# yakir1991/LoRa-SDR-Lightweight-Standalone-Library-

Hardware: AMD Instinct MI355X
Metric: Msymbols/s dechirp+FFT+argmax @ SF7 & SF12, 1/2/4/8 GPU; % HBM roofline (higher is better)
Workload: dtype f32; 1 GPU; SF7 BW125 osr1 LEGACY lora_demodulate + fused dechirp, 15625 frames x (2 sync + 64 data) symbols per GPU, noiseless; launch=eager, streams=3, sf=7, osr=1, frames_per_gpu=15625, data_symbols_per_frame=64, parallelism=frames sharded x1, no collective (gloo timing only), symbols_ok=True

## Files before the change

lora-sdr-lightweight-standalone-library-_amd/csrc/lora_demod_fast.hip:

```cpp
#include "../../include/lora_mi355x.h"
#include "lora_internal.h"

#include <algorithm>
#include <cstdlib>
#include <type_traits>
#include <utility>

#pragma clang fp contract(off)

namespace lora {
namespace {


template <int SF>
struct Geo {
  static constexpr int N = 1 << SF;
  static constexpr bool SMALL = SF <= 5;
  static constexpr int P = SMALL ? N : 16;
  static constexpr int T = N / P;
  static constexpr int R1 = SMALL ? N : ((SF & 1) ? 8 : 16);
  static constexpr int LOGR1 = SMALL ? SF : ((SF & 1) ? 3 : 4);
  static constexpr int G1 = P / R1;
  static constexpr bool R2FIRST = (SF & 1) != 0;
  static constexpr int X = N / R1;
// ... 468 lines not shown
    case 0: return cf{1.0f, 0.0f};
    case 1: return cf{C1, -S1};
    case 2: return cf{R2, -R2};
    case 3: return cf{S1, -C1};
    case 4: return cf{0.0f, -1.0f};
    case 5: return cf{-S1, -C1};
    case 6: return cf{-R2, -R2};
    case 7: return cf{-C1, -S1};
    case 8: return cf{-1.0f, 0.0f};
    default: return cf{-C1, S1};
  }
}
template <int N>
struct ConstTw1 {
  __device__ __forceinline__ cf operator[](int i) const { return w16(i / (N / 16)); }
};

template <int SF, bool KEEP, bool FMA = false, bool TWL = false, bool PACK = false, bool CPRE = false,
          class HOOK = NoHook, bool FOLD = false>
__device__ __forceinline__ uint64_t fft_key(cf* z, cf* row, int l, const KArgs& a, float* second = nullptr,
                                            const cf* twl = nullptr, const int* cpre = nullptr, HOOK hook = HOOK{},
                                            const cf* wbpre = nullptr, const cf* wfold = nullptr) {
  using G = Geo<SF>;
  constexpr int N = G::N, T = G::T, P = G::P, R1 = G::R1;
  constexpr bool WL = G::WAVE_LOCAL;
  static_assert(!FOLD || FMA, "the folded rotation is the certified path's");
#pragma unroll
  for (int h = 0; h < G::G1; ++h) {
    if constexpr (FOLD) {
      cf* x = z + h * R1;
      const cf* w = wfold + h * R1;
      if constexpr (G::R2FIRST) {
#pragma unroll
        for (int b = 0; b < R1; b += 2) bfly2<true>(x[b], x[b + 1], w[b + 1]);
      } else {
#pragma unroll
        for (int b = 0; b < R1; b += 4) bfly4<true>(x[b], x[b + 1], x[b + 2], x[b + 3], w[b + 1], w[b + 2], w[b + 3]);
      }
      pass_regs<R1, G::R2FIRST, N, 1, !KEEP, FMA, ConstTw1<N>, true>(x, 0, ConstTw1<N>{});
    } else if constexpr (FMA) {
      pass_regs<R1, G::R2FIRST, N, 1, !KEEP, FMA, ConstTw1<N>>(z + h * R1, 0, ConstTw1<N>{});
    } else {
      pass_regs<R1, G::R2FIRST, N, 1, !KEEP, FMA>(z + h * R1, 0, a.tw);
    }
  }
  uint64_t key = 0;
  if constexpr (G::NPASS == 1) {
    float best = 0.0f;
    uint32_t bi = 0;
#pragma unroll
    for (int u = 0; u < R1; ++u) {
      const float m2 = z[u].re * z[u].re + z[u].im * z[u].im;
      if (m2 > best) {
        best = m2;
        bi = (uint32_t)u;
      }
    }
    key = ((uint64_t)__float_as_uint(best) << 32) | (uint32_t)(~bi);
  } else {
    int c[G::G1];
#pragma unroll
    for (int h = 0; h < G::G1; ++h) c[h] = CPRE ? cpre[h] : (int)(a.rev[l + T * h] >> G::LOGR1);
#pragma unroll
    for (int h = 0; h < G::G1; ++h)
#pragma unroll
      for (int u = 0; u < R1; ++u)
        row[lds_slot<SF>(c[h] * R1) + u] = z[h * R1 + u];
    block_sync<WL>();
    constexpr int RL = G::NPASS == 2 ? G::RA : G::RB;
    constexpr int ML = G::NPASS == 2 ? G::MA_A : G::MA_B;
    const cf* twA = TWL ? twl : a.twTA;
    if constexpr (G::NPASS == 2) {
      pass_lds<G::RA, N, G::MA_A, SF, T, P, true, FMA, false, TWL, PACK>(row, z, l, a.tw, key, twA, second);
    } else {
      pass_lds<G::RA, N, G::MA_A, SF, T, P, false, FMA, false, TWL>(row, z, l, a.tw, key, twA);
      block_sync<WL>();
      write_pass<G::RA, G::MA_A, SF, T, P>(row, z, l);
      block_sync<WL>();
      if constexpr (!std::is_same_v<HOOK, NoHook>) {
        const cf* wb = wbpre;
        __builtin_amdgcn_sched_barrier(0);
        hook();
        __builtin_amdgcn_sched_barrier(0);
        pass_lds<G::RB, N, G::MA_B, SF, T, P, true, FMA, true, TWL, PACK>(row, z, l, a.tw, key, a.twTB2, second, wb);
      } else {
        pass_lds<G::RB, N, G::MA_B, SF, T, P, true, FMA, true, TWL, PACK>(row, z, l, a.tw, key, a.twTB2, second);
      }
    }
    if constexpr (KEEP) {
      block_sync<WL>();
#pragma unroll
      for (int gg = 0; gg < P / RL; ++gg)
#pragma unroll
        for (int u = 0; u < RL; ++u) row[lds_slot<SF>(l + T * gg) + lds_slot<SF>(ML * u)] = z[gg * RL + u];
      block_sync<WL>();
    }
  }
  return key;
}

template <int SF, bool KEEP>
__device__ __forceinline__ void fft_key2(cf* z0, cf* z1, cf* row0, cf* row1, int l, const KArgs& a,
                                         uint64_t& k0, uint64_t& k1) {
  using G = Geo<SF>;
  static_assert(G::NPASS == 2 && G::WAVE_LOCAL, "wave-local two-pass transforms only");
  constexpr int N = G::N, T = G::T, P = G::P, R1 = G::R1;
#pragma unroll
  for (int h = 0; h < G::G1; ++h) {
    pass_regs<R1, G::R2FIRST, N, 1, !KEEP>(z0 + h * R1, 0, a.tw);
    pass_regs<R1, G::R2FIRST, N, 1, !KEEP>(z1 + h * R1, 0, a.tw);
  }
  int c[G::G1];
#pragma unroll
  for (int h = 0; h < G::G1; ++h) c[h] = (int)(a.rev[l + T * h] >> G::LOGR1);
#pragma unroll
  for (int h = 0; h < G::G1; ++h)
#pragma unroll
    for (int u = 0; u < R1; ++u) {
      row0[lds_slot<SF>(c[h] * R1) + u] = z0[h * R1 + u];
      row1[lds_slot<SF>(c[h] * R1) + u] = z1[h * R1 + u];
    }
  wave_sync();
  pass_lds<G::RA, N, G::MA_A, SF, T, P, true>(row0, z0, l, a.tw, k0, a.twTA);
  pass_lds<G::RA, N, G::MA_A, SF, T, P, true>(row1, z1, l, a.tw, k1, a.twTA);
  if constexpr (KEEP) {
    wave_sync();
#pragma unroll
    for (int gg = 0; gg < P / G::RA; ++gg)
#pragma unroll
      for (int u = 0; u < G::RA; ++u) {
        row0[lds_slot<SF>(l + T * gg) + lds_slot<SF>(G::MA_A * u)] = z0[gg * G::RA + u];
        row1[lds_slot<SF>(l + T * gg) + lds_slot<SF>(G::MA_A * u)] = z1[gg * G::RA + u];
      }
    wave_sync();
  }
}

template <int SF>
__device__ __forceinline__ uint64_t symbol_key(uint64_t key, int tid, uint64_t* red) {
  constexpr int T = Geo<SF>::T;
  if constexpr (T <= 64) {
    return group_max(key, T);
  } else {
    key = group_max(key, 64);
    __syncthreads();
    if ((tid & 63) == 0) red[tid >> 6] = key;
    __syncthreads();
    constexpr int WPS = T / 64;
    const int wb = ((tid >> 6) / WPS) * WPS;
    uint64_t r = red[wb];
#pragma unroll
    for (int q = 1; q < WPS; ++q) r = umax64(r, red[wb + q]);
    return r;
  }
}

__device__ __forceinline__ float amax3(float m, cf v) {
  asm("v_max3_f32 %0, %0, |%1|, |%2|" : "+v"(m) : "v"(v.re), "v"(v.im));
  return m;
}

template <int SF>
__device__ __forceinline__ void group_reduce2(float& a, float& b, int tid, float* rf) {
  constexpr int T = Geo<SF>::T;
  constexpr int W = T < 64 ? T : 64;
#pragma unroll
  for (int o = W >> 1; o > 0; o >>= 1) {
    a = fmaxf(a, __shfl_xor(a, o, 64));
    b = fmaxf(b, __shfl_xor(b, o, 64));
  }
  if constexpr (T > 64) {
    const int w = tid >> 6;
    if ((tid & 63) == 0) {
      rf[2 * w] = a;
      rf[2 * w + 1] = b;
    }
    __syncthreads();
    constexpr int WPS = T / 64;
    const int wb = (w / WPS) * WPS;
    a = rf[2 * wb];
    b = rf[2 * wb + 1];
#pragma unroll
    for (int q = 1; q < WPS; ++q) {
      a = fmaxf(a, rf[2 * (wb + q)]);
      b = fmaxf(b, rf[2 * (wb + q) + 1]);
    }
  }
}

__device__ __forceinline__ void top2_merge(uint32_t& b, uint32_t& s, uint32_t& p, uint32_t b2, uint32_t s2,
                                           uint32_t p2) {
  const uint32_t lo = b < b2 ? b : b2;
  const uint32_t hs = s > s2 ? s : s2;
  s = hs > lo ? hs : lo;
  b = b > b2 ? b : b2;
  p = p > p2 ? p : p2;
}
template <int O>
__device__ __forceinline__ uint32_t dpp_xchg(uint32_t v) {
  constexpr int ctrl = O == 1 ? 0xB1 : O == 2 ? 0x4E : O == 4 ? 0x141 : 0x140;
  return (uint32_t)__builtin_amdgcn_mov_dpp((int)v, ctrl, 0xF, 0xF, true);
}
template <int O, int W>
__device__ __forceinline__ void spec_reduce_step(uint32_t& best, uint32_t& sec, uint32_t& pm) {
  if constexpr (O < W) {
    if constexpr (O <= 8) {
      top2_merge(best, sec, pm, dpp_xchg<O>(best), dpp_xchg<O>(sec), dpp_xchg<O>(pm));
    } else if constexpr (O == 16) {
      const auto xb = __builtin_amdgcn_permlane16_swap(best, best, false, false);
      const auto xs = __builtin_amdgcn_permlane16_swap(sec, sec, false, false);
      const auto xp = __builtin_amdgcn_permlane16_swap(pm, pm, false, false);
      best = xb[0], sec = xs[0], pm = xp[0];
      top2_merge(best, sec, pm, xb[1], xs[1], xp[1]);
    } else {
      static_assert(O == 32, "wave64");
      const auto xb = __builtin_amdgcn_permlane32_swap(best, best, false, false);
      const auto xs = __builtin_amdgcn_permlane32_swap(sec, sec, false, false);
      const auto xp = __builtin_amdgcn_permlane32_swap(pm, pm, false, false);
      best = xb[0], sec = xs[0], pm = xp[0];
      top2_merge(best, sec, pm, xb[1], xs[1], xp[1]);
    }
    spec_reduce_step<2 * O, W>(best, sec, pm);
  }
}
template <int SF>
__device__ __forceinline__ void spec_reduce(uint32_t& best, uint32_t& sec, float& pmf, int tid, uint32_t* scratch) {
  constexpr int T = Geo<SF>::T;
  uint32_t pm = __float_as_uint(pmf);
  spec_reduce_step<1, (T < 64 ? T : 64)>(best, sec, pm);
  if constexpr (T > 64) {
    const int w = tid >> 6;
    if ((tid & 63) == 0) {
      scratch[3 * w] = best;
      scratch[3 * w + 1] = sec;
      scratch[3 * w + 2] = pm;
    }
    __syncthreads();
    constexpr int WPS = T / 64;
    const int wb = (w / WPS) * WPS;
    best = scratch[3 * wb];
    sec = scratch[3 * wb + 1];
    pm = scratch[3 * wb + 2];
#pragma unroll
    for (int q = 1; q < WPS; ++q)
      top2_merge(best, sec, pm, scratch[3 * (wb + q)], scratch[3 * (wb + q) + 1], scratch[3 * (wb + q) + 2]);
  }
  pmf = __uint_as_float(pm);
}

template <int SF>
constexpr int demod_waves_per_eu() {
  return SF >= 6 ? 4 : 1;
}

template <int SF, bool SPEC>
constexpr int demod_twl_entries() {
  if constexpr (!SPEC || SF < 6) {
    return 0;
  } else {
    using G = Geo<SF>;
    return (G::RA == 16 ? 15 : 3) * G::MA_A;
  }
}


template <int SF>
constexpr size_t spec_dtl_offset() {
  return (((size_t)Geo<SF>::SPW * lds_row<SF>() + demod_twl_entries<SF, true>()) * sizeof(cf) + 15) & ~(size_t)15;
}
template <int SF>
constexpr bool spec_dtab() {
  return Geo<SF>::WAVE_LOCAL && Geo<SF>::NPASS == 2 &&
         4 * (spec_dtl_offset<SF>() + 2 * sizeof(cf) * Geo<SF>::N) <= 160 * 1024;
}
template <int SF>
constexpr size_t spec_lds_bytes() {
  constexpr bool pf2 = Geo<SF>::WAVE_LOCAL && Geo<SF>::NPASS == 2;
  return pf2 ? spec_dtl_offset<SF>() + (spec_dtab<SF>() ? 2 * sizeof(cf) * Geo<SF>::N : 16 * 8 * Geo<SF>::T)
             : sizeof(cf) * ((size_t)Geo<SF>::SPW * lds_row<SF>() + demod_twl_entries<SF, true>());
}

#define LORA_SPEC_BLOCKS(SPB, dblocks, frames, sync) ((dblocks) + ((sync) ? (2 * (frames) + (SPB) - 1) / (SPB) : 0))
template <int SF>
struct SpecGrid {
  static constexpr int SPB = Geo<SF>::WAVE_LOCAL ? 64 / Geo<SF>::T : Geo<SF>::SPW;
  static constexpr int BPG = Geo<SF>::WAVE_LOCAL ? 4 : 1;
  __host__ __device__ static constexpr int bpf(int per) { return (per + SPB - 1) / SPB; }
  static constexpr int64_t groups(int64_t frames, int per, bool sync) {
    return (LORA_SPEC_BLOCKS(SPB, frames * bpf(per), frames, sync) + BPG - 1) / BPG;
  }
};

__device__ __forceinline__ __amdgpu_buffer_rsrc_t raw_rsrc(const void* p) {
  return __builtin_amdgcn_make_buffer_rsrc(const_cast<void*>(p), (short)0, 0x7fffffff, 0x00020000);
}

struct SpecBlk {
  int64_t f, base;
  int s, jl, d, cg;
  bool valid, mis, nbr;
  float rate;
  int toff;
};
template <int SF, int SPM, int DW, bool RECIP>
__device__ __forceinline__ void spec_decode(const KArgs& a, int64_t bb, int bpf, int per, int gi, int l, bool fdiv,
                                            uint64_t mq, SpecBlk& B) {
  constexpr int SPB = SpecGrid<SF>::SPB, S0 = SPM == 2 ? 0 : 2;
  const __attribute__((address_space(4))) FrameParams* fps =
      (const __attribute__((address_space(4))) FrameParams*)a.fp_spec;
  if constexpr (RECIP)
    B.f = fdiv ? (bpf == 1 ? bb : (int64_t)(((uint64_t)(uint32_t)bb * mq) >> 32)) : bb / bpf;
  else
    B.f = bb / bpf;
  B.jl = (int)(bb - B.f * bpf) * SPB + gi;
  B.valid = B.jl < per;
  B.s = S0 + (B.valid ? B.jl : per - 1);
  B.rate = SPM == 2 ? 0.0f : fps[B.f].rate;
  B.toff = SPM == 2 ? 0 : fps[B.f].t_off;
  sym_base(B.s, Geo<SF>::N, a.frame_len, B.toff, B.base, B.cg);
  if constexpr (SPM == 1) B.cg = 0;
  B.d = (int)(B.base & (DW - 1));
  B.mis = __builtin_amdgcn_readfirstlane(__ballot(Geo<SF>::NPASS == 3 ? l < B.d : B.d != 0) != 0);
  B.nbr = false;
}
template <int SF>
__device__ __forceinline__ bool spec_next_is_neighbour(const KArgs& a, const SpecBlk& B, int per, int gi) {
  int64_t bnext;
  int cgn;
  sym_base(B.s + 1, Geo<SF>::N, a.frame_len, B.toff, bnext, cgn);
  return gi < SpecGrid<SF>::SPB - 1 && B.jl + 1 < per && bnext == B.base + Geo<SF>::N;
}

template <int SF, bool DTAB, bool DTL>
__device__ __forceinline__ float4 spec_table_pair(int pp, __amdgpu_buffer_rsrc_t rd, int vt, bool cg0, const cf* dq,
                                                  const float4* dl) {
  constexpr int N = Geo<SF>::N, T = Geo<SF>::T;
  if constexpr (DTAB) {
    const cf d0 = dq[2 * pp * T], d1 = dq[(2 * pp + 1) * T];
    return float4{d0.re, d0.im, d1.re, d1.im};
  } else if constexpr (DTL) {
    return cg0 ? dl[pp * T]
               : __builtin_bit_cast(float4, __builtin_amdgcn_raw_buffer_load_b128(rd, vt, pp * (N + T) * 16, 0));
  } else {
    return __builtin_bit_cast(float4, __builtin_amdgcn_raw_buffer_load_b128(rd, vt, pp * (N + T) * 16, 0));
  }
}
template <int SF, bool DTAB, bool DTL, int NP>
__device__ __forceinline__ void spec_table(const KArgs& a, int cg, int lr, const cf* dtab, const float4* dtl,
                                           float4 (&dt)[NP]) {
  const __amdgpu_buffer_rsrc_t rd = raw_rsrc(a.downP);
  const int vt = (cg + lr) * 16;
  bool cg0 = false;
  if constexpr (DTL && !DTAB) cg0 = __builtin_amdgcn_readfirstlane(__ballot(cg != 0) == 0);
#pragma unroll
  for (int pp = 0; pp < NP; ++pp) dt[pp] = spec_table_pair<SF, DTAB, DTL>(pp, rd, vt, cg0, dtab + cg + lr, dtl + lr);
}
template <int MODE, bool MAX, int P>
__device__ __forceinline__ float spec_dechirp_max(const v2f (&ld)[P + 1], const float4* dt, cf (&in)[P]) {
#pragma unroll
  for (int q = 0; q < P; ++q) in[q] = cf{ld[q].x, ld[q].y};
  if constexpr (MODE == 0) {
#pragma unroll
    for (int pp = 0; pp < P / 2; ++pp) {
      in[2 * pp] = pk_cmul_ref(in[2 * pp], cf{dt[pp].x, dt[pp].y});
      in[2 * pp + 1] = pk_cmul_ref(in[2 * pp + 1], cf{dt[pp].z, dt[pp].w});
    }
  }
  float pm = 0.0f;
  if constexpr (MAX) {
#pragma unroll
    for (int q = 0; q < P; ++q) pm = amax3(pm, in[q]);
  }
  return pm;
}

__device__ __forceinline__ float spec_margin(uint32_t best, uint32_t sec) {
  return __builtin_amdgcn_sqrtf(spec_key_value(best)) - __builtin_amdgcn_sqrtf(spec_key_value(sec));
}
template <int SF, int S0>
__device__ __forceinline__ void spec_store_symbol(const KArgs& a, int64_t f, int s, int l, int lr, uint32_t lbest,
                                                  uint32_t best, uint32_t sec, float pm) {
  using G = Geo<SF>;
  constexpr int NG = G::NPASS == 2 ? G::P / G::RA : G::P / G::RB;
  constexpr int ML = G::NPASS == 2 ? G::MA_A : G::MA_B;
  const int o = (int)(best & 15u);
  const uint32_t idx = (uint32_t)(lr + G::T * (o % NG) + ML * (o / NG));
  const float margin = spec_margin(best, sec);
  if (lbest == best && a.syms) a.syms[f * a.sym_stride + (s - S0)] = (uint16_t)idx;
  if (l == 0)
    reinterpret_cast<uint2*>(a.spec_marg)[f * a.total + s] = make_uint2(__float_as_uint(margin), __float_as_uint(pm));
}

template <int SF, int MODE, bool FAST = false, bool SPEC = false>
__global__ void __launch_bounds__(256) __attribute__((amdgpu_waves_per_eu(demod_waves_per_eu<SF>())))
k_demod_fast(KArgs a, int s0, int64_t work, int rowc) {
  using G = Geo<SF>;
  constexpr int N = G::N, T = G::T, P = G::P, SPW = G::SPW;
  constexpr bool RAW = MODE == 3;
  constexpr bool DYN = MODE >= 2;
  extern __shared__ __attribute__((aligned(16))) unsigned char smem[];
  __shared__ uint64_t red[4];
  cf* rows = reinterpret_cast<cf*>(smem);
  const int tid = threadIdx.x;
  const int per = a.total - s0;
  const int step = DYN ? a.step : N;
  const int osr = DYN ? a.osr : 1;
  const bool legacy = RAW ? true : DYN ? a.mode != LORA_MODE_API : true;
  const bool dech = DYN ? (legacy && a.dechirp) : (MODE == 0);
  const bool hann = DYN ? (a.hann != 0) : false;

  const int g = tid / T;
  const int l = tid % T;
  const int64_t w0 = (int64_t)blockIdx.x * SPW;
  const int64_t f0 = w0 / per;
  const int r0 = (int)(w0 - f0 * per);
  const int64_t w = w0 + g;
  const bool valid = w < work;
  const int loc = r0 + (int)((valid ? w : work - 1) - w0);
  const int q = per >= SPW ? (loc >= per ? 1 : 0) : (int)((unsigned)loc / (unsigned)per);
  const int64_t f = f0 + q;
  const int s = s0 + (loc - q * per);
  const FrameParams p = RAW ? FrameParams{0.0f, 0.0f, 0.0f, 1.0f, 0, 0, 0, 0} : (SPEC ? a.fp_spec[f] : a.fp[f]);
  int64_t base;
  int cg;
  sym_base(s, step, a.frame_len, p.t_off, base, cg);
  const cf* __restrict__ x = a.iq + f * a.frame_stride + base;
  const float start = p.rate * ((float)((uint32_t)s * (uint32_t)N) + (float)p.t_off / (float)osr);
  const float scale = (legacy && p.scaled) ? p.scale : 1.0f;

  constexpr bool FMA = SPEC && FAST;
  constexpr int NTW = demod_twl_entries<SF, SPEC>();
  static_assert(NTW <= 256, "one staged twiddle per thread");
  cf* twl = rows + (size_t)SPW * rowc;
  cf tv{0.0f, 0.0f};
  if constexpr (NTW > 0) {
    if (tid < NTW) tv = a.twTA ? a.twTA[tid] : a.tw[twT_index(N, G::MA_A, tid / G::MA_A, tid % G::MA_A)];
  }
  cf in[P], z[P];
  if (SPEC && MODE == 0 && a.downP)
    gather_points<SF, true>(a, x, l, 1, N, cg, 1, true, 1.0f, in);
  else
    gather_points<SF>(a, x, l, osr, step, cg, legacy ? 1 : 2, dech, SPEC ? 1.0f : scale, in);
  if constexpr (NTW > 0) {
    if (tid < NTW) twl[tid] = tv;
    if constexpr (G::WAVE_LOCAL) __syncthreads();
  }
  float pm = 0.0f;
  if constexpr (SPEC) {
#pragma unroll
    for (int q = 0; q < P; ++q) pm = amax3(pm, in[q]);
  }
  rotate_place<SF, !RAW, FAST, FMA>(in, z, start, p.rate, hann, a.win, l);
  if constexpr (SPEC) asm volatile("" : "+v"(pm));
  float sec = 0.0f;
  const uint64_t lkey =
      fft_key<SF, false, FMA, (NTW > 0)>(z, rows + (size_t)g * rowc, l, a, SPEC ? &sec : nullptr, twl);
  const uint64_t key = symbol_key<SF>(lkey, tid, red);
  if (l == 0 && valid && a.syms) a.syms[f * a.sym_stride + (s - s0)] = (uint16_t)key_index(key);
  if constexpr (SPEC) {
    float r2 = lkey == key ? sec : key_value(lkey);
    group_reduce2<SF>(r2, pm, tid, reinterpret_cast<float*>(smem + 64));
    if (l == 0 && valid) {
      const int64_t per = a.total - s0;
      reinterpret_cast<float2*>(a.spec_marg)[f * per + (s - s0)] = make_float2(sqrtf(key_value(key)) - sqrtf(r2), pm);
    }
  }
}


template <int SF, int MODE, bool HANN = false, int OSRV = 1, int SPM = 0>
__global__ void __launch_bounds__(256) __attribute__((amdgpu_waves_per_eu(demod_waves_per_eu<SF>())))
k_spec_demod(KArgs a, int64_t frames, int rowc, int64_t gstride) {
  using G = Geo<SF>;
  constexpr int N = G::N, T = G::T, P = G::P, SPW = G::SPW;
  constexpr bool WL = G::WAVE_LOCAL;
  using SG = SpecGrid<SF>;
  constexpr int SPB = SG::SPB;
  constexpr int BPG = SG::BPG;
  constexpr int NTW = demod_twl_entries<SF, true>();
  constexpr bool OSRN = OSRV != 1;
  constexpr bool FOLD = SF <= 8 && !HANN;
  static_assert(P == 16 && (MODE == 0 || MODE == 1), "SF >= 6, LEGACY (osr 1, or OSRN)");
  static_assert(OSRV == 0 || OSRV == 1 || OSRV == 2 || OSRV == 4, "osr 1, 2, 4 or run time");
  static_assert(NTW <= 256, "one staged twiddle per thread");
  extern __shared__ __attribute__((aligned(16))) unsigned char smem[];
  __shared__ uint32_t red3[3 * 4];
  cf* rows = reinterpret_cast<cf*>(smem);
  cf* twl = rows + (size_t)SPW * rowc;
  const int tot = a.total;
  constexpr bool API = SPM == 1, RAWM = SPM == 2;
  constexpr int S0 = RAWM ? 0 : 2;
  const int per = tot - S0;
  constexpr bool DTL = WL && G::NPASS == 2 && !OSRN && MODE == 0;
  constexpr bool DTAB = DTL && spec_dtab<SF>();
  float4* dtl = reinterpret_cast<float4*>(smem + spec_dtl_offset<SF>());
  cf* dtab = reinterpret_cast<cf*>(smem + spec_dtl_offset<SF>());
  if (SPM != 0 && blockIdx.x == 0 && threadIdx.x < kFixStripes) a.fix_count[16 * threadIdx.x] = 0;
  if constexpr (NTW > 0) {
    const int tid = threadIdx.x;
    if (tid < NTW) twl[tid] = a.twTA ? a.twTA[tid] : a.tw[twT_index(N, G::MA_A, tid / G::MA_A, tid % G::MA_A)];
    if constexpr (DTAB) {
      for (int i = tid; i < 2 * N; i += 256) dtab[i] = a.down[i];
    } else if constexpr (DTL) {
      static_assert(8 * T <= 256, "one staged pair per thread");
      if (tid < 8 * T) dtl[tid] = reinterpret_cast<const float4*>(a.downP)[(tid / T) * (N + T) + tid % T];
    }
    __syncthreads();
  }
  const int bpf = SG::bpf(per);
  const int64_t dblocks = frames * bpf;
  const int64_t blocks = LORA_SPEC_BLOCKS(SPB, dblocks, frames, SPM == 0);
  const int64_t groups = (blocks + BPG - 1) / BPG;
  const int wave = __builtin_amdgcn_readfirstlane((int)(threadIdx.x >> 6));

  auto run_block = [&](auto sync_c, int64_t b, int64_t fb, int rb) {
    constexpr bool SYNC = decltype(sync_c)::value;
    int tid = threadIdx.x;
    asm volatile("" : "+v"(tid));
    const int g = SPW == 1 ? 0 : tid / T;
    const int l = tid % T;
    const int gi = WL ? (g % SPB) : g;
    int64_t f, fu;
    int s;
    bool valid;
    int rel = 0;
    if constexpr (!SYNC) {
      f = fu = fb;
      const int jl = rb * SPB + gi;
      valid = jl < per;
      s = S0 + (valid ? jl : per - 1);
    } else {
      const int64_t k0 = (b - dblocks) * SPB;
      int64_t k = k0 + gi;
      valid = k < 2 * frames;
      if (!valid) k = 2 * frames - 1;
      f = k >> 1;
      s = (int)(k & 1);
      fu = k0 >> 1;
      rel = (int)((f - fu) * a.frame_stride * 8);
    }
    const FrameParams fp = RAWM ? FrameParams{} : a.fp_spec[f];
    const float rate = RAWM ? 0.0f : fp.rate;
    const int toff = RAWM ? 0 : fp.t_off;
    const int step = OSRN ? a.step : N;
    int64_t base;
    int cg;
    sym_base(s, step, a.frame_len, toff, base, cg);
    if constexpr (API) cg = 0;
    cf in[P];
    float pm = 0.0f;
    int lr = l;
    if constexpr (OSRN) {
      const int osr = OSRV ? OSRV : a.osr;
      const __amdgpu_buffer_rsrc_t rx = raw_rsrc(a.iq + fu * a.frame_stride);
      const __amdgpu_buffer_rsrc_t rd = raw_rsrc(a.down);
      const int vo = rel + (int)(base + (int64_t)l * osr) * 8;
      const int vt = (cg + l * osr) * 8;
      const int so = T * osr * 8;
      if constexpr (OSRV == 4) {
        const bool odd = (l & 1) != 0;
        lr = odd ? T / 2 + (l >> 1) : (l >> 1);
        const int vo2 = rel + (int)base * 8 + 16 * l;
        const int vt2 = (cg + 2 * l) * 8;
#pragma unroll
        for (int q = 0; q < P; ++q) {
          cf e0;
#pragma unroll
          for (int h = 0; h < 2; ++h) {
            const int i = 2 * q + h;
            const float4 y2 = __builtin_bit_cast(float4, __builtin_amdgcn_raw_buffer_load_b128(rx, vo2, i * 2 * T * 8, 2 ));
            cf y0 = cf{y2.x, y2.y}, y1 = cf{y2.z, y2.w};
            if constexpr (MODE == 0) {
              const float4 d2 = __builtin_bit_cast(float4, __builtin_amdgcn_raw_buffer_load_b128(rd, vt2, i * 2 * T * 8, 0));
              y0 = pk_cmul_ref(y0, cf{d2.x, d2.y});
              y1 = pk_cmul_ref(y1, cf{d2.z, d2.w});
            }
            if constexpr (!SYNC) pm = amax3(amax3(pm, y0), y1);
            if (h == 0) {
              e0 = y0;
            } else {
              const cf m = cf{__int_as_float(__builtin_amdgcn_update_dpp(0, __float_as_int(y0.re), 0x111, 0xF, 0xF, false)),
                              __int_as_float(__builtin_amdgcn_update_dpp(0, __float_as_int(y0.im), 0x111, 0xF, 0xF, false))};
              in[q] = odd ? m : e0;
            }
          }
        }
      } else if constexpr (OSRV == 2) {
#pragma unroll
        for (int q = 0; q < P; ++q) {
          const float4 y2 = __builtin_bit_cast(float4, __builtin_amdgcn_raw_buffer_load_b128(rx, vo, q * so, 2 ));
          cf y0 = cf{y2.x, y2.y}, y1 = cf{y2.z, y2.w};
          if constexpr (MODE == 0) {
            const float4 d2 = __builtin_bit_cast(float4, __builtin_amdgcn_raw_buffer_load_b128(rd, vt, q * so, 0));
            y0 = pk_cmul_ref(y0, cf{d2.x, d2.y});
            y1 = pk_cmul_ref(y1, cf{d2.z, d2.w});
          }
          if constexpr (!SYNC) pm = amax3(amax3(pm, y0), y1);
          in[q] = y0;
        }
      } else {
#pragma unroll
      for (int q = 0; q < P; ++q) {
        for (int k = 0; k < osr; ++k) {
          cf y = __builtin_bit_cast(cf, __builtin_amdgcn_raw_buffer_load_b64(rx, vo + 8 * k, q * so, 2 ));
          if constexpr (MODE == 0)
            y = pk_cmul_ref(y, __builtin_bit_cast(cf, __builtin_amdgcn_raw_buffer_load_b64(rd, vt + 8 * k, q * so, 0)));
          if constexpr (!SYNC) pm = amax3(pm, y);
          if (k == 0) in[q] = y;
        }
      }
      }
    } else {
    constexpr int D = T < 8 ? T : 8;
    const int d = (int)(base & (D - 1));
    lr = (l - d) & (T - 1);
    v2f ld[P + 1];
    const __amdgpu_buffer_rsrc_t rx = raw_rsrc(a.iq + fu * a.frame_stride);
    const int vo = rel + (int)(base - d + l) * 8;
    float4 dt[MODE == 0 ? P / 2 : 1];
    const __amdgpu_buffer_rsrc_t rd = raw_rsrc(a.downP);
    const int vt = (cg + lr) * 16;
    constexpr int AUX = SYNC ? 0 : 2;
#pragma unroll
    for (int pp = 0; pp < P / 2; ++pp) {
      if constexpr (MODE == 0) dt[pp] = spec_table_pair<SF, false, false>(pp, rd, vt, false, nullptr, nullptr);
#pragma unroll
      for (int q = 2 * pp; q < 2 * pp + 2; ++q)
        ld[q] = __builtin_bit_cast(v2f, __builtin_amdgcn_raw_buffer_load_b64(rx, vo, q * T * 8, AUX));
    }
    if (__builtin_amdgcn_readfirstlane(__ballot(l < d) != 0)) {
      const bool late = l < d;
      ld[P] = __builtin_bit_cast(
          v2f, __builtin_amdgcn_raw_buffer_load_b64(rx, late ? vo : vo - T * 8, P * T * 8, AUX));
#pragma unroll
      for (int q = 0; q < P; ++q) ld[q] = late ? ld[q + 1] : ld[q];
    }
    pm = spec_dechirp_max<MODE, !SYNC>(ld, dt, in);
    }
    cf z[P], wz[P];
    {
      v2f F[P];
      spec_factors<SF>(rate, lr, F);
      spec_rotate_place<SF, HANN, FOLD>(in, z, F, a.win, lr, wz);
    }
    asm volatile("" : "+v"(pm));
    const uint64_t lk = fft_key<SF, false, true, (NTW > 0), true, false, NoHook, FOLD>(
        z, rows + (size_t)g * rowc, lr, a, nullptr, twl, nullptr, NoHook{}, nullptr, wz);
    const uint32_t lbest = (uint32_t)lk;
    uint32_t best = lbest, sec = (uint32_t)(lk >> 32);
    spec_reduce<SF>(best, sec, pm, tid, red3);
    if (valid) {
      constexpr int NG = (G::NPASS == 2 ? P / G::RA : P / G::RB);
      constexpr int ML = G::NPASS == 2 ? G::MA_A : G::MA_B;
      const int o = (int)(best & 15u);
      const uint32_t idx = (uint32_t)(lr + T * (o % NG) + ML * (o / NG));
      const float margin = spec_margin(best, sec);
      uint2* mg = reinterpret_cast<uint2*>(a.spec_marg) + f * tot + s;
      if constexpr (!SYNC) {
        if (lbest == best && a.syms) a.syms[f * a.sym_stride + (s - S0)] = (uint16_t)idx;
        if (l == 0) *mg = make_uint2(__float_as_uint(margin), __float_as_uint(pm));
      } else {
        if (lbest == best) *mg = make_uint2(__float_as_uint(margin), idx);
      }
    }
    block_sync<WL>();
  };
  int64_t grp0 = blockIdx.x;
  constexpr bool PL = SF == 7 && !HANN && WL && G::NPASS == 2 && !OSRN;
  const int64_t bstep = gstride * BPG;
  if constexpr (PL) {
    static_assert(T == 8 && P == 16 && G::G1 == 2 && G::R1 == 8 && G::LOGR1 == 3 && FOLD, "SF7 geometry");
    static_assert(MODE != 0 || (DTAB && NTW > 0), "the fused dechirp reads the staged doubled table");
    constexpr int DL = 16;
    const int tid0 = threadIdx.x;
    const int g = tid0 / T;
    const int l = tid0 % T;
    const int gi = g % SPB;
    float4 nx[P / 2 + 1];
    const bool fdiv = (uint64_t)dblocks * (uint64_t)bpf < (1ull << 32);
    const uint64_t mq = ((1ull << 32) + (uint64_t)bpf - 1) / (uint64_t)bpf;
    auto issue = [&](int64_t bb, SpecBlk& B) {
      spec_decode<SF, SPM, DL, true>(a, bb, bpf, per, gi, l, fdiv, mq, B);
      const __amdgpu_buffer_rsrc_t rx = raw_rsrc(a.iq + B.f * a.frame_stride);
      const int vo = (int)(B.base - B.d) * 8 + 16 * l;
#pragma unroll
      for (int j = 0; j < P / 2; ++j)
        nx[j] = __builtin_bit_cast(float4, __builtin_amdgcn_raw_buffer_load_b128(rx, vo, j * DL * 8, 2 ));
      if (B.mis) {
        B.nbr = spec_next_is_neighbour<SF>(a, B, per, gi);
        if (!B.nbr) {
          if (2 * l < B.d) {
            const v2f e0 = __builtin_bit_cast(v2f, __builtin_amdgcn_raw_buffer_load_b64(rx, vo, (P / 2) * DL * 8, 2));
            nx[P / 2].x = e0.x;
            nx[P / 2].y = e0.y;
          }
          if (2 * l + 1 < B.d) {
            const v2f e1 = __builtin_bit_cast(v2f, __builtin_amdgcn_raw_buffer_load_b64(rx, vo + 8, (P / 2) * DL * 8, 2));
            nx[P / 2].z = e1.x;
            nx[P / 2].w = e1.y;
          }
        }
      }
    };
    int64_t b = grp0 * BPG + wave;
    SpecBlk nb{};
    if (b < dblocks) issue(b, nb);
    for (; b < dblocks; b += bstep, grp0 += gstride) {
      const SpecBlk B = nb;
      float4(&ld)[P / 2 + 1] = nx;
      const int d = B.d;
      int r[2];
      bool late[2];
#pragma unroll
      for (int h = 0; h < 2; ++h) {
        const int x = 2 * l + h - d;
        late[h] = x < 0;
        r[h] = x & (DL - 1);
      }
      cf dv[MODE == 0 ? P : 1];
      if constexpr (MODE == 0) {
#pragma unroll
        for (int h = 0; h < 2; ++h) {
          const cf* dq = dtab + B.cg + r[h];
#pragma unroll
          for (int m = 0; m < P / 2; ++m) dv[h + 2 * m] = dq[DL * m];
        }
      }
      cf in[P];
      if (B.mis) {
        const int src = ((int)__lane_id() + T) & 63;
        const float4 n0 = {__shfl(ld[0].x, src, 64), __shfl(ld[0].y, src, 64), __shfl(ld[0].z, src, 64),
                           __shfl(ld[0].w, src, 64)};
        if (B.nbr) ld[P / 2] = n0;
#pragma unroll
        for (int m = 0; m < P / 2; ++m) {
          in[2 * m] = late[0] ? cf{ld[m + 1].x, ld[m + 1].y} : cf{ld[m].x, ld[m].y};
          in[2 * m + 1] = late[1] ? cf{ld[m + 1].z, ld[m + 1].w} : cf{ld[m].z, ld[m].w};
        }
      } else {
#pragma unroll
        for (int m = 0; m < P / 2; ++m) {
          in[2 * m] = cf{ld[m].x, ld[m].y};
          in[2 * m + 1] = cf{ld[m].z, ld[m].w};
        }
      }
      constexpr bool EARLY = MODE == 0;
      if constexpr (EARLY) {
        __builtin_amdgcn_sched_barrier(0);
        if (b + bstep < dblocks) issue(b + bstep, nb);
        __builtin_amdgcn_sched_barrier(0);
      }
      if constexpr (MODE == 0) {
#pragma unroll
        for (int q = 0; q < P; ++q) in[q] = pk_cmul_ref(in[q], dv[q]);
      }
      float pm = 0.0f;
#pragma unroll
      for (int q = 0; q < P; ++q) pm = amax3(pm, in[q]);
      asm volatile("" : "+v"(pm));
      cf z[P], wz[P];
      {
        v2f F[P];
        spec_factors_pl(B.rate, r, F);
        spec_rotate_place<SF, false, FOLD>(in, z, F, a.win, l, wz);
      }
      asm volatile("" : "+v"(pm));
      if constexpr (!EARLY) {
        __builtin_amdgcn_sched_barrier(0);
        if (b + bstep < dblocks) issue(b + bstep, nb);
        __builtin_amdgcn_sched_barrier(0);
      }
      int cpre[2];
#pragma unroll
      for (int h = 0; h < 2; ++h) cpre[h] = ((r[h] & 3) << 2) | (r[h] >> 2);
      const uint64_t lk = fft_key<SF, false, true, (NTW > 0), true, true, NoHook, FOLD>(
          z, rows + (size_t)g * rowc, l, a, nullptr, twl, cpre, NoHook{}, nullptr, wz);
      const uint32_t lbest = (uint32_t)lk;
      uint32_t best = lbest, sec = (uint32_t)(lk >> 32);
      spec_reduce<SF>(best, sec, pm, tid0, red3);
      if (B.valid) spec_store_symbol<SF, S0>(a, B.f, B.s, l, l, lbest, best, sec, pm);
      wave_sync();
    }
  }
  constexpr bool PF8 = !OSRN && !PL;
  if constexpr (PF8) {
    constexpr bool P3 = G::NPASS == 3;
    static_assert(P3 || (WL && G::NPASS == 2), "two-pass geometries are wave-local");
    constexpr int D = T < 8 ? T : 8;
    const int tid0 = threadIdx.x;
    const int g = SPW == 1 ? 0 : tid0 / T;
    const int l = tid0 % T;
    const int gi = WL ? g % SPB : g;
    const int lane0 = (int)(__lane_id()) - l;
    int cown[G::G1];
#pragma unroll
    for (int h = 0; h < G::G1; ++h) cown[h] = (int)(a.rev[l + T * h] >> G::LOGR1);
    v2f nx[P + 1];
    auto issue = [&](int64_t bb, SpecBlk& B) {
      spec_decode<SF, SPM, D, false>(a, bb, bpf, per, gi, l, false, 0, B);
      const __amdgpu_buffer_rsrc_t rx = raw_rsrc(a.iq + B.f * a.frame_stride);
      const int vo = (int)(B.base - B.d + l) * 8;
#pragma unroll
      for (int q = 0; q < P; ++q)
        nx[q] = __builtin_bit_cast(v2f, __builtin_amdgcn_raw_buffer_load_b64(rx, vo, q * T * 8, 2 ));
      if (B.mis) {
        if constexpr (P3) {
          nx[P] = __builtin_bit_cast(
              v2f, __builtin_amdgcn_raw_buffer_load_b64(rx, l < B.d ? vo : vo - T * 8, P * T * 8, 2 ));
        } else {
          B.nbr = spec_next_is_neighbour<SF>(a, B, per, gi);
          if (l < B.d && !B.nbr)
            nx[P] = __builtin_bit_cast(v2f, __builtin_amdgcn_raw_buffer_load_b64(rx, vo, P * T * 8, 2 ));
        }
      }
    };
    int64_t b = grp0 * BPG + (WL ? wave : 0);
    SpecBlk nb{};
    if (b < dblocks) issue(b, nb);
    for (; b < dblocks; b += bstep, grp0 += gstride) {
      const SpecBlk B = nb;
      v2f(&ld)[P + 1] = nx;
      const int d = B.d;
      const int lr = (l - d) & (T - 1);
      float4 dt[MODE == 0 ? P / 2 : 1];
      if constexpr (MODE == 0) spec_table<SF, DTAB, DTL>(a, B.cg, lr, dtab, dtl, dt);
      if (B.mis) {
        const bool late = l < d;
        if constexpr (!P3) {
          const int src = ((int)__lane_id() + T) & 63;
          const v2f n0 = {__shfl(ld[0].x, src, 64), __shfl(ld[0].y, src, 64)};
          if (late && B.nbr) ld[P] = n0;
        }
#pragma unroll
        for (int q = 0; q < P; ++q) ld[q] = late ? ld[q + 1] : ld[q];
      }
      cf in[P];
      float pm = spec_dechirp_max<MODE, true>(ld, dt, in);
      constexpr int NTB = G::RB == 16 ? 15 : 3;
      cf wb[P3 ? (P / G::RB) * NTB : 1];
      if constexpr (P3) {
#pragma unroll
        for (int gg = 0; gg < P / G::RB; ++gg) load_tw2<G::RB, G::MA_B>(wb + gg * NTB, (lr + T * gg) % G::MA_B, a.twTB2);
      }
      asm volatile("" : "+v"(pm));
      cf z[P], wz[P];
      {
        v2f F[P];
        spec_factors<SF>(B.rate, lr, F);
        spec_rotate_place<SF, HANN, FOLD>(in, z, F, a.win, lr, wz);
      }
      asm volatile("" : "+v"(pm));
      auto prefetch = [&]() {
        if (b + bstep < dblocks) issue(b + bstep, nb);
      };
      int cpre[G::G1];
      uint64_t lk;
      if constexpr (P3) {
#pragma unroll
        for (int h = 0; h < G::G1; ++h) cpre[h] = d == 0 ? cown[h] : (int)(a.rev[lr + T * h] >> G::LOGR1);
        lk = fft_key<SF, false, true, (NTW > 0), true, true, decltype(prefetch), FOLD>(
            z, rows + (size_t)g * rowc, lr, a, nullptr, twl, cpre, prefetch, wb, wz);
      } else {
        __builtin_amdgcn_sched_barrier(0);
        prefetch();
        __builtin_amdgcn_sched_barrier(0);
#pragma unroll
        for (int h = 0; h < G::G1; ++h) cpre[h] = __shfl(cown[h], lane0 + lr, 64);
        lk = fft_key<SF, false, true, (NTW > 0), true, true, NoHook, FOLD>(
            z, rows + (size_t)g * rowc, lr, a, nullptr, twl, cpre, NoHook{}, nullptr, wz);
      }
      const uint32_t lbest = (uint32_t)lk;
      uint32_t best = lbest, sec = (uint32_t)(lk >> 32);
      spec_reduce<SF>(best, sec, pm, tid0, red3);
      if (B.valid) spec_store_symbol<SF, S0>(a, B.f, B.s, l, lr, lbest, best, sec, pm);
      block_sync<WL>();
    }
  }
  for (int64_t grp = grp0; grp < groups; grp += gstride) {
    const int64_t b = grp * BPG + (WL ? wave : 0);
    if (WL && b >= blocks) break;
    if (b < dblocks) {
      const int64_t fb = b / bpf;
      run_block(std::false_type{}, b, fb, (int)(b - fb * bpf));
    } else {
      run_block(std::true_type{}, b, 0, 0);
    }
  }
}

template <int SF>
struct EstGeo {
  static constexpr int T = Geo<SF>::T;
  static constexpr int BLOCK = T >= 64 ? 256 : 64;
  static constexpr int SPB = BLOCK / T;
  static constexpr bool PAIR = SF >= 7 && Geo<SF>::WAVE_LOCAL && Geo<SF>::NPASS == 2;
};

template <int SF, int MODE>
__device__ __forceinline__ uint32_t exact_symbol(const KArgs& a, const cf* __restrict__ x,
                                                           const FrameParams& q, int s, cf* row, int l, int tid,
                                                           uint64_t* red) {
  using G = Geo<SF>;
  constexpr int N = G::N, P = G::P;
  constexpr bool DYN = MODE == 2;
  const int step = DYN ? a.step : N;
  const int osr = DYN ? a.osr : 1;
  const bool legacy = DYN ? a.mode != LORA_MODE_API : true;
  const bool dech = DYN ? (legacy && a.dechirp) : (MODE == 0);
  const bool hann = a.hann != 0;
  int64_t base;
  int cg;
  sym_base(s, step, a.frame_len, q.t_off, base, cg);
  const float start = q.rate * ((float)((uint32_t)s * (uint32_t)N) + (float)q.t_off / (float)osr);
  cf in[P], z[P];
  gather_points<SF>(a, x + base, l, osr, step, cg, legacy ? 1 : 2, dech, (legacy && q.scaled) ? q.scale : 1.0f, in);
  rotate_place<SF, true>(in, z, start, q.rate, hann, a.win, l);
  uint64_t key = fft_key<SF, false>(z, row, l, a);
  key = symbol_key<SF>(key, tid, red);
  block_sync<G::WAVE_LOCAL>();
  return key_index(key);
}

constexpr double kHwSinCosErr = 2.0e-7;

template <int SF, int LANES>
__device__ __forceinline__ void certify_list(const KArgs& a, int64_t f, const FrameParams& q, bool valid, int li) {
  constexpr int N = 1 << SF;
  const FrameParams qs = a.fp_spec[f];
  const int per = a.total - 2;
  const bool same_t = qs.t_off == q.t_off;
  constexpr int T = N >= 16 ? N / 16 : 1;
  const double u = 1.0 / 16777216.0;
  const double E = (8.0 * SF + 42.0) * u;
  const double drate = fabs((double)q.rate - (double)qs.rate);
  const double rmax = fmax(fabs((double)q.rate), fabs((double)qs.rate));
  const double tabs = (double)abs(q.t_off);
  const double e_spec = 36.0 * u * rmax * T + 16.0 * (1.87e-7 + 1.4143 * kHwSinCosErr) + 2.6e-6 + 9.6e-7;
  auto certified = [&](double d, double wmax, int s) {
    const double n1 = 2.0 * N * wmax;
    const double L = (double)(s + 1) * N + tabs;
    const double e_ref = u * rmax * (L + 2.0 * N);
    const double B = n1 * (drate * N + e_ref + e_spec + 2.0 * E);
    return same_t && d > 4.0 * B + 0x1p-60;
  };
  const uint2* __restrict__ mg = reinterpret_cast<const uint2*>(a.spec_marg) + f * a.total;
  bool sync_rej = false;
  if (a.mode != LORA_MODE_API) {
    const uint2 e = mg[li < 2 ? li : 0];
    const bool ok = certified((double)__uint_as_float(e.x), (double)__uint_as_float(a.maxbits[f]), li & 1);
    const uint32_t ok1 = (uint32_t)__shfl_down((int)ok, 1, 64), i1 = (uint32_t)__shfl_down((int)e.y, 1, 64);
    if (li == 0 && valid) {
      if (ok && ok1) {
        if (a.sync) {
          const unsigned shift = a.sf > 4 ? a.sf - 4 : 0;
          a.sync[f] = (uint8_t)((((e.y >> shift) & 0x0f) << 4) | ((i1 >> shift) & 0x0f));
        }
      } else {
        sync_rej = true;
      }
    }
  }
  if (valid) {
    uint64_t rejbits = 0;
#pragma unroll 8
    for (int j = li, k = 0; j < per; j += LANES, ++k) {
      const uint2 v = mg[2 + j];
      if (!certified((double)__uint_as_float(v.x), (double)__uint_as_float(v.y), 2 + j)) rejbits |= 1ull << k;
    }
    const int rounds = (per + LANES - 1) / LANES;
    unsigned total = 0;
    for (int k = 0; k <= rounds; ++k)
      total += (unsigned)__popcll(__ballot(k < rounds ? ((rejbits >> k) & 1) != 0 : sync_rej));
    if (total) {
      const int lane = (int)__lane_id();
      const int first = __builtin_ctzll(__ballot(1));
      const int stripe = (int)(blockIdx.x % kFixStripes);
      unsigned base = 0;
      if (lane == first) base = atomicAdd(a.fix_count + 16 * stripe, total);
      base = (unsigned)__shfl((int)base, first, 64);
      uint32_t* list = a.fix_list + 2 * (size_t)stripe * (size_t)a.fix_cap;
      for (int k = 0; k <= rounds; ++k) {
        const bool rej = k < rounds ? ((rejbits >> k) & 1) != 0 : sync_rej;
        const uint64_t m = __ballot(rej);
        if (rej) {
          const size_t slot = base + (unsigned)__popcll(m & ((1ull << lane) - 1));
          list[2 * slot] = (uint32_t)f;
          list[2 * slot + 1] = k < rounds ? (uint32_t)(li + LANES * k) : 0xFFFFFFFFu;
        }
        base += (unsigned)__popcll(m);
      }
    }
  }
}

constexpr int est_waves_per_eu(int SF, int MODE, int SPEC) {
  if (SF < 10) return 2;
  if (SPEC == 1) return MODE == 2 ? 3 : 4;
  if (SPEC == 2) return SF == 11 ? 3 : 4;
  return 2;
}

template <int SF, int MODE, int SPEC = 0>
__global__ void __launch_bounds__(256) __attribute__((amdgpu_waves_per_eu(est_waves_per_eu(SF, MODE, SPEC))))
k_est_fast(KArgs a, int64_t frames, int rowc) {
  using G = Geo<SF>;
  constexpr int N = G::N, T = G::T, P = G::P;
  constexpr int SPB = (T >= 64 ? 256 : 64) / T;
  constexpr bool DYN = MODE == 2;
  extern __shared__ __attribute__((aligned(16))) unsigned char smem[];
  __shared__ uint64_t red[4];
  __shared__ FrameParams sp[SPB];
  const int tid = threadIdx.x;
  if (SPEC == 1 && blockIdx.x == 0 && tid < kFixStripes) a.fix_count[16 * tid] = 0;
  const int step = DYN ? a.step : N;
  const int osr = DYN ? a.osr : 1;
  const bool legacy = DYN ? a.mode != LORA_MODE_API : true;
  const bool dech = DYN ? (legacy && a.dechirp) : (MODE == 0);
  const bool hann = (DYN || SPEC != 0) ? (a.hann != 0) : false;
  const int g = tid / T;
  const int l = tid % T;
  const int64_t f0 = (int64_t)blockIdx.x * SPB + g;
  const bool valid = f0 < frames;
  const int64_t f = valid ? f0 : frames - 1;
  const cf* __restrict__ x = a.iq + f * a.frame_stride;
  cf* row = reinterpret_cast<cf*>(smem) + (size_t)g * rowc;
  float maxv = 0.0f;
  if (legacy && SPEC != 1) {
    if constexpr (SPEC == 2) {
      maxv = __uint_as_float(a.maxbits[f]);
      const int per = a.total - 2;
      const float2* __restrict__ mg = reinterpret_cast<const float2*>(a.spec_marg) + f * a.total + 2;
#pragma unroll 8
      for (int j = l; j < per; j += T) maxv = fmaxf(maxv, mg[j].y);
    } else {
      for (int c = l; c < a.mx_bpf; c += T) maxv = fmaxf(maxv, __uint_as_float(a.maxbits[f * a.mx_bpf + c]));
    }
    maxv = __uint_as_float((uint32_t)(symbol_key<SF>((uint64_t)__float_as_uint(maxv) << 32, tid, red) >> 32));
  }
  const int scaled = maxv > 1.0f;
  const float scale = scaled ? 1.0f / maxv : 1.0f;
  if constexpr (SPEC == 2) {
    if (!scaled) {
      if (l == 0 && valid) {
        const FrameParams qs = load_fp(a.fp_spec + f);
        store_fp(a.fp + f, qs);
        if (a.cfo) a.cfo[f] = qs.cfo;
        if (a.toff) a.toff[f] = qs.toff;
        if (a.max_amp) a.max_amp[f] = maxv;
      }
    }
  }
  FrameParams q;
  if (SPEC == 2 && !scaled) {
    q = a.fp_spec[f];
  } else {

    float sum_index = 0.0f, phase_diff = 0.0f, prev_phase = 0.0f;
    bool have_prev = false;
    unsigned sum_t = 0;
    cf in[P], z[P];
    float mo = 0.0f;
    constexpr bool PAIR = EstGeo<SF>::PAIR && MODE <= 1;
    if constexpr (PAIR) {
      cf* row1 = row + (size_t)EstGeo<SF>::SPB * rowc;
      cf in1[P], z1[P];
      float bp[2] = {-1e30f, -1e30f}, bfi[2] = {0.0f, 0.0f};
      uint32_t bidx[2] = {0, 0};
      unsigned bt[2] = {0, 0};
      cf bbin[2] = {cf{0.0f, 0.0f}, cf{0.0f, 0.0f}};
      for (int t = 0; t < osr; ++t) {
        gather_points<SF>(a, x + t, l, osr, step, t, legacy ? 1 : 0, dech, scale, in);
        gather_points<SF>(a, x + (int64_t)step + t, l, osr, step, t, legacy ? 1 : 0, dech, scale, in1);
        if constexpr (SPEC == 1) {
#pragma unroll
          for (int q = 0; q < P; ++q) mo = amax3(amax3(mo, in[q]), in1[q]);
          asm volatile("" : "+v"(mo));
        }
        rotate_place<SF, false>(in, z, 0.0f, 0.0f, hann, a.win, l);
        rotate_place<SF, false>(in1, z1, 0.0f, 0.0f, hann, a.win, l);
        uint64_t key[2];
        fft_key2<SF, true>(z, z1, row, row1, l, a, key[0], key[1]);
        key[0] = group_max(key[0], T);
        key[1] = group_max(key[1], T);
        if (l == 0) {
#pragma unroll
          for (int s = 0; s < 2; ++s) {
            const cf* rw = s ? row1 : row;
            const uint32_t idx = key_index(key[s]);
            const uint32_t im1 = idx > 0 ? idx - 1 : N - 1, ip1 = idx < (uint32_t)N - 1 ? idx + 1 : 0;
            const cf L = rw[lds_slot<SF>((int)im1)], R = rw[lds_slot<SF>((int)ip1)],
                     B = rw[lds_slot<SF>((int)idx)];
            float pw, fi;
            detect_tail(key_value(key[s]), L, R, a.power_scale, &pw, &fi);
            if (pw > bp[s] || (legacy && pw == bp[s] && idx < bidx[s])) {
              bp[s] = pw;
              bidx[s] = idx;
              bfi[s] = fi;
              bt[s] = (unsigned)t;
              bbin[s] = B;
            }
          }
        }
        wave_sync();
      }
      if (l == 0) {
#pragma unroll
        for (int s = 0; s < 2; ++s) {
          sum_t += bt[s];
          sum_index += (float)bidx[s] + bfi[s];
          const float phase = lm_atan2f(bbin[s].im, bbin[s].re);
          if (have_prev) {
            float d = phase - prev_phase;
            while (d > PI_F) d -= 2.0f * PI_F;
            while (d < -PI_F) d += 2.0f * PI_F;
            phase_diff += d;
          }
          prev_phase = phase;
          have_prev = true;
        }
      }
    }
    for (int s = 0; s < (PAIR ? 0 : 2); ++s) {
      float best_p = -1e30f, best_fi = 0.0f;
      uint32_t best_idx = 0;
      unsigned best_t = 0;
      cf best_bin = {0.0f, 0.0f};
      for (int t = 0; t < osr; ++t) {
        int lo = l;
        asm volatile("" : "+v"(lo));
        gather_points<SF>(a, x + (int64_t)s * step + t, lo, osr, step, t, legacy ? 1 : 0, dech,
                             scale, in);
        if constexpr (SPEC == 1) {
#pragma unroll
          for (int q = 0; q < P; ++q) mo = amax3(mo, in[q]);
          asm volatile("" : "+v"(mo));
        }
        rotate_place<SF, false>(in, z, 0.0f, 0.0f, hann, a.win, lo);
        uint64_t key = fft_key<SF, true>(z, row, lo, a);
        key = symbol_key<SF>(key, tid, red);
        if (l == 0) {
          const uint32_t idx = key_index(key);
          const uint32_t im1 = idx > 0 ? idx - 1 : N - 1, ip1 = idx < (uint32_t)N - 1 ? idx + 1 : 0;
          cf L, R, B;
          if constexpr (G::NPASS == 1) {
            L = R = B = cf{0.0f, 0.0f};
#pragma unroll
            for (int u = 0; u < N; ++u) {
              if ((uint32_t)u == im1) L = z[u];
              if ((uint32_t)u == ip1) R = z[u];
              if ((uint32_t)u == idx) B = z[u];
            }
          } else {
            L = row[lds_slot<SF>((int)im1)];
            R = row[lds_slot<SF>((int)ip1)];
            B = row[lds_slot<SF>((int)idx)];
          }
// ... 620 lines not shown
```

Measured before the change: 5350 Msymbols/s.

## Prefetch frame params one block ahead and defer shared-table staging past first load

Splits per-block decode into a frame-parameter fetch (frame index, rate, timing offset from constant memory) and a placement step. The fetch for the block after next is issued one iteration ahead, so its scalar latency no longer sits in front of the IQ buffer loads. Twiddle and dechirp table staging into LDS is split into a register load and a later store. The store and its barrier now happen after the first IQ loads are issued, so the prologue overlaps global latency. The cost is more live registers, and some configurations (SF9 raw, SF8 Hann, three-pass) are excluded to avoid spills.

```diff
diff --git a/lora-sdr-lightweight-standalone-library-_amd/csrc/lora_demod_fast.hip b/lora-sdr-lightweight-standalone-library-_amd/csrc/lora_demod_fast.hip
--- a/lora-sdr-lightweight-standalone-library-_amd/csrc/lora_demod_fast.hip
+++ b/lora-sdr-lightweight-standalone-library-_amd/csrc/lora_demod_fast.hip
@@ -794,21 +794,32 @@
   float rate;
   int toff;
 };
-template <int SF, int SPM, int DW, bool RECIP>
-__device__ __forceinline__ void spec_decode(const KArgs& a, int64_t bb, int bpf, int per, int gi, int l, bool fdiv,
-                                            uint64_t mq, SpecBlk& B) {
-  constexpr int SPB = SpecGrid<SF>::SPB, S0 = SPM == 2 ? 0 : 2;
+struct SpecFetch {
+  int64_t f;
+  float rate;
+  int toff;
+};
+template <int SF, int SPM, bool RECIP>
+__device__ __forceinline__ void spec_fetch(const KArgs& a, int64_t bb, int bpf, bool fdiv, uint64_t mq, SpecFetch& F) {
   const __attribute__((address_space(4))) FrameParams* fps =
       (const __attribute__((address_space(4))) FrameParams*)a.fp_spec;
   if constexpr (RECIP)
-    B.f = fdiv ? (bpf == 1 ? bb : (int64_t)(((uint64_t)(uint32_t)bb * mq) >> 32)) : bb / bpf;
+    F.f = fdiv ? (bpf == 1 ? bb : (int64_t)(((uint64_t)(uint32_t)bb * mq) >> 32)) : bb / bpf;
   else
-    B.f = bb / bpf;
+    F.f = bb / bpf;
+  F.rate = SPM == 2 ? 0.0f : fps[F.f].rate;
+  F.toff = SPM == 2 ? 0 : fps[F.f].t_off;
+}
+template <int SF, int SPM, int DW>
+__device__ __forceinline__ void spec_place(const KArgs& a, const SpecFetch& F, int64_t bb, int bpf, int per, int gi,
+                                           int l, SpecBlk& B) {
+  constexpr int SPB = SpecGrid<SF>::SPB, S0 = SPM == 2 ? 0 : 2;
+  B.f = F.f;
   B.jl = (int)(bb - B.f * bpf) * SPB + gi;
   B.valid = B.jl < per;
   B.s = S0 + (B.valid ? B.jl : per - 1);
-  B.rate = SPM == 2 ? 0.0f : fps[B.f].rate;
-  B.toff = SPM == 2 ? 0 : fps[B.f].t_off;
+  B.rate = F.rate;
+  B.toff = F.toff;
   sym_base(B.s, Geo<SF>::N, a.frame_len, B.toff, B.base, B.cg);
   if constexpr (SPM == 1) B.cg = 0;
   B.d = (int)(B.base & (DW - 1));
@@ -988,17 +999,45 @@
   float4* dtl = reinterpret_cast<float4*>(smem + spec_dtl_offset<SF>());
   cf* dtab = reinterpret_cast<cf*>(smem + spec_dtl_offset<SF>());
   if (SPM != 0 && blockIdx.x == 0 && threadIdx.x < kFixStripes) a.fix_count[16 * threadIdx.x] = 0;
-  if constexpr (NTW > 0) {
-    const int tid = threadIdx.x;
-    if (tid < NTW) twl[tid] = a.twTA ? a.twTA[tid] : a.tw[twT_index(N, G::MA_A, tid / G::MA_A, tid % G::MA_A)];
-    if constexpr (DTAB) {
-      for (int i = tid; i < 2 * N; i += 256) dtab[i] = a.down[i];
-    } else if constexpr (DTL) {
-      static_assert(8 * T <= 256, "one staged pair per thread");
-      if (tid < 8 * T) dtl[tid] = reinterpret_cast<const float4*>(a.downP)[(tid / T) * (N + T) + tid % T];
-    }
-    __syncthreads();
-  }
+  constexpr int NDT = DTAB ? (2 * N + 255) / 256 : 1;
+  cf stw{}, sdt[NDT] = {};
+  float4 sdl{};
+  auto stage_load = [&]() {
+    if constexpr (NTW > 0) {
+      const int tid = threadIdx.x;
+      if (tid < NTW) stw = a.twTA ? a.twTA[tid] : a.tw[twT_index(N, G::MA_A, tid / G::MA_A, tid % G::MA_A)];
+      if constexpr (DTAB) {
+#pragma unroll
+        for (int k = 0; k < NDT; ++k)
+          if (tid + 256 * k < 2 * N) sdt[k] = a.down[tid + 256 * k];
+      } else if constexpr (DTL) {
+        static_assert(8 * T <= 256, "one staged pair per thread");
+        if (tid < 8 * T) sdl = reinterpret_cast<const float4*>(a.downP)[(tid / T) * (N + T) + tid % T];
+      }
+    }
+  };
+  auto stage_store = [&]() {
+    if constexpr (NTW > 0) {
+      const int tid = threadIdx.x;
+      if (tid < NTW) twl[tid] = stw;
+      if constexpr (DTAB) {
+#pragma unroll
+        for (int k = 0; k < NDT; ++k)
+          if (tid + 256 * k < 2 * N) dtab[tid + 256 * k] = sdt[k];
+      } else if constexpr (DTL) {
+        if (tid < 8 * T) dtl[tid] = sdl;
+      }
+      __syncthreads();
+    }
+  };
+  constexpr bool SPILLS_BOTH = SF == 9 && RAWM, SPILLS_AHEAD = SF == 8 && HANN && MODE == 0;
+  constexpr bool AHEAD = !SPILLS_BOTH && !SPILLS_AHEAD && G::NPASS != 3;
+  constexpr bool FIRST = !OSRN && !SPILLS_BOTH;
+  stage_load();
+  if constexpr (!FIRST) stage_store();
+  auto stage_late = [&]() {
+    if constexpr (FIRST) stage_store();
+  };
   const int bpf = SG::bpf(per);
   const int64_t dblocks = frames * bpf;
   const int64_t blocks = LORA_SPEC_BLOCKS(SPB, dblocks, frames, SPM == 0);
@@ -1171,8 +1210,9 @@
     float4 nx[P / 2 + 1];
     const bool fdiv = (uint64_t)dblocks * (uint64_t)bpf < (1ull << 32);
     const uint64_t mq = ((1ull << 32) + (uint64_t)bpf - 1) / (uint64_t)bpf;
-    auto issue = [&](int64_t bb, SpecBlk& B) {
-      spec_decode<SF, SPM, DL, true>(a, bb, bpf, per, gi, l, fdiv, mq, B);
+    auto fetch = [&](int64_t bb, SpecFetch& F) { spec_fetch<SF, SPM, true>(a, bb, bpf, fdiv, mq, F); };
+    auto request = [&](int64_t bb, const SpecFetch& F, SpecBlk& B) {
+      spec_place<SF, SPM, DL>(a, F, bb, bpf, per, gi, l, B);
       const __amdgpu_buffer_rsrc_t rx = raw_rsrc(a.iq + B.f * a.frame_stride);
       const int vo = (int)(B.base - B.d) * 8 + 16 * l;
 #pragma unroll
@@ -1196,7 +1236,25 @@
     };
     int64_t b = grp0 * BPG + wave;
     SpecBlk nb{};
-    if (b < dblocks) issue(b, nb);
+    SpecFetch nf{};
+    auto issue = [&](int64_t bb) {
+      if constexpr (!AHEAD) fetch(bb, nf);
+      request(bb, nf, nb);
+    };
+    auto fetch_after = [&](int64_t bb) {
+      if constexpr (AHEAD) {
+        if (bb + bstep < dblocks) fetch(bb + bstep, nf);
+      }
+    };
+    if (b < dblocks) {
+      if constexpr (AHEAD) fetch(b, nf);
+      issue(b);
+      fetch_after(b);
+      stage_late();
+      asm volatile("");
+    } else {
+      stage_late();
+    }
     for (; b < dblocks; b += bstep, grp0 += gstride) {
       const SpecBlk B = nb;
       float4(&ld)[P / 2 + 1] = nx;
@@ -1239,12 +1297,17 @@
       constexpr bool EARLY = MODE == 0;
       if constexpr (EARLY) {
         __builtin_amdgcn_sched_barrier(0);
-        if (b + bstep < dblocks) issue(b + bstep, nb);
+        if (b + bstep < dblocks) issue(b + bstep);
         __builtin_amdgcn_sched_barrier(0);
       }
       if constexpr (MODE == 0) {
 #pragma unroll
         for (int q = 0; q < P; ++q) in[q] = pk_cmul_ref(in[q], dv[q]);
+      }
+      if constexpr (EARLY) {
+        __builtin_amdgcn_sched_barrier(0);
+        fetch_after(b + bstep);
+        __builtin_amdgcn_sched_barrier(0);
       }
       float pm = 0.0f;
 #pragma unroll
@@ -1259,7 +1322,8 @@
       asm volatile("" : "+v"(pm));
       if constexpr (!EARLY) {
         __builtin_amdgcn_sched_barrier(0);
-        if (b + bstep < dblocks) issue(b + bstep, nb);
+        if (b + bstep < dblocks) issue(b + bstep);
+        fetch_after(b + bstep);
         __builtin_amdgcn_sched_barrier(0);
       }
       int cpre[2];
@@ -1288,8 +1352,9 @@
 #pragma unroll
     for (int h = 0; h < G::G1; ++h) cown[h] = (int)(a.rev[l + T * h] >> G::LOGR1);
     v2f nx[P + 1];
-    auto issue = [&](int64_t bb, SpecBlk& B) {
-      spec_decode<SF, SPM, D, false>(a, bb, bpf, per, gi, l, false, 0, B);
+    auto fetch = [&](int64_t bb, SpecFetch& F) { spec_fetch<SF, SPM, false>(a, bb, bpf, false, 0, F); };
+    auto request = [&](int64_t bb, const SpecFetch& F, SpecBlk& B) {
+      spec_place<SF, SPM, D>(a, F, bb, bpf, per, gi, l, B);
       const __amdgpu_buffer_rsrc_t rx = raw_rsrc(a.iq + B.f * a.frame_stride);
       const int vo = (int)(B.base - B.d + l) * 8;
 #pragma unroll
@@ -1308,7 +1373,22 @@
     };
     int64_t b = grp0 * BPG + (WL ? wave : 0);
     SpecBlk nb{};
-    if (b < dblocks) issue(b, nb);
+    SpecFetch nf{};
+    auto issue = [&](int64_t bb) {
+      if constexpr (!AHEAD) fetch(bb, nf);
+      request(bb, nf, nb);
+      if constexpr (AHEAD) {
+        if (bb + bstep < dblocks) fetch(bb + bstep, nf);
+      }
+    };
+    if (b < dblocks) {
+      if constexpr (AHEAD) fetch(b, nf);
+      issue(b);
+      stage_late();
+      asm volatile("");
+    } else {
+      stage_late();
+    }
     for (; b < dblocks; b += bstep, grp0 += gstride) {
       const SpecBlk B = nb;
       v2f(&ld)[P + 1] = nx;
@@ -1343,7 +1423,7 @@
       }
       asm volatile("" : "+v"(pm));
       auto prefetch = [&]() {
-        if (b + bstep < dblocks) issue(b + bstep, nb);
+        if (b + bstep < dblocks) issue(b + bstep);
       };
       int cpre[G::G1];
       uint64_t lk;
```

Result: no change. 5343 Msymbols/s (-0.1%).
